# bistoyek21-ric/StrikeForce

Measured on AMD Instinct MI355X. Metric: env-steps/sec (whole node), 64x64 map x32 entities, higher is better.
Workload: dtype int32

## Files before the change

strikeforce_amd/csrc/sf_core.hpp:

```cpp
#pragma once
#include "../../include/strikeforce.h"
#include "sf_types.hpp"

#if defined(SF_EXP_FAKE_DRAWS) && !defined(SF_EXPERIMENT_BUILD)
#error "SF_EXP_FAKE_DRAWS makes draw() return wrong numbers on purpose (tools/experiments/r03_rows): timing builds only, together with -DSF_EXPERIMENT_BUILD"
#endif

namespace sf {

enum { SH_WALL, SH_HUMAN, SH_ZOMBIE, SH_PUP, SH_PDN, SH_BULLET, SH_CHEST, SH_POUT, SH_EMPTY };
enum { LIM_PORTAL = 1000, LIM_BLOCK = 1100 };

#define SF_SHAPE(f) (SH::FIXED ? SH::f(p) : p.f)
constexpr uint32_t mod5_frac(uint32_t x) { return (x * 205u) & 1023u; }
constexpr bool mod5_frac_exact() {
  for (uint32_t x = 0; x < 1024u; ++x)
    if ((x % 5u < 2u) != (mod5_frac(x) < 410u) || (x % 5u < 3u) != (mod5_frac(x) < 615u)) return false;
  return true;
}
static_assert(mod5_frac_exact(), "x % 5 < 2 and x % 5 < 3 by the fraction's bits, for every x < 1024");
#define SF_MOD5_LT(x, n) (SH::FIXED ? mod5_frac(x) < ((n) == 2u ? 410u : 615u) : mod5(x) < (n))
template <class W, int NB, bool HBM_PLANE = false, bool BITMAPS = !HBM_PLANE, bool ZL = false, class SH = RuntimeShape>
struct Core {
  using V = typename W::V;
  using P = typename W::P;

  struct Arena {
    V hpos, hfl, hhp, hst, hmd, hk, hdm, hef, hc01, hc23, ht01, ht23, hbpk, hcmd;
    V zpos, zhp, zmd;
    uint32_t *zl;
    uint32_t zcap;
    uint32_t zwn;
    uint32_t zwhi;
    uint32_t *pl;
    uint32_t pwn, pwhi;
    V ba[NB], bd[NB], bb[NB], bc[NB];
    V ppos;
    V rl, rus, rseed;
    V rl2, rseed2;
    uint32_t warm;
    uint32_t wrate;
    const uint32_t *xt;
    const uint32_t *ht;
    uint32_t *bm;
    V la;
    V la2;
    uint32_t la2_ok;
    int32_t frame, kills, tkills, loot, chests, steps, episodes, done, outcome, ended;
    int32_t fph;
    uint32_t jomle;
    uint32_t tb_lo, tb_hi, sr_lo, sr_hi;
    uint32_t dirty;
    uint32_t pd01, pd23, pd45;
#ifdef SF_DIAG_STAMPS
    V dacc;
    uint32_t dlast;
#endif
  };

  static constexpr uint32_t RL_ZERO = 0x10000u;
  static SF_DEV V mod65537_v(V x) {
    const V t = (x & 0xffffu) - (x >> 16);
    return W::minu(t, t + 65537u);
  }
  static SF_DEV V pow3_v(const uint32_t *xt, V m, P pred) {
    return mod65537_v(W::lds_u32(xt, m & 255u, pred) * W::lds_u32(xt + 256, m >> 8, pred));
  }

  template <bool WANT_OUT>
  static SF_DEV V draw_core(V &rl, const V &rus, const V &rseed, uint32_t &jomle, const uint32_t *xt, const Params &p) {
    const P tap = W::ltu(W::lane(), 18u) & ((rl & RL_ZERO) == 0u);
    const V pw = pow3_v(xt, (rl * rseed) & 0xffffu, tap);
    const V sum = W::sum18_row1(W::select(tap, rus * pw, V(0u))) + 1u;
    V t = mod65537_v(sum);
    t = W::select(t == 0u, V(1u), t);
    jomle += 1u;
    const uint32_t e = jomle & 0xffffu;
    const V lg = W::gload_u16(p.logt, t + (uint32_t)LOGT_OFF, W::all());
    const V lnew = (lg * e) & 0xffffu;
    rl = W::select(W::lane() == 17u, lnew, W::shl1(rl));
    if (WANT_OUT) return pow3_v(xt, lnew, W::all()) & 1023u;
    return V(0u);
  }
  static constexpr uint32_t SUM_BIAS_LANE = 63489u + 11u * 65537u;
  static_assert((32ull * SUM_BIAS_LANE) % 65537ull == 1ull, "the lanes' bias must add up to the generator's +1");
  static_assert(SUM_BIAS_LANE % 2u == 0u, "it is also a byte offset into a table of 16-bit entries");
  static_assert(16ull * SUM_BIAS_LANE > 16ull * 10ull * 65536ull, "a row's partial sum must stay positive");
  static_assert((32ull * SUM_BIAS_LANE + 18ull * 10ull * 65535ull) >> 16 < (unsigned long long)LOGT_OFF, "index below the table");
  static SF_DEV const uint16_t *log_base(const Params &p) { return p.logt + LOGT_OFF - (int)(SUM_BIAS_LANE / 2u); }
  static SF_DEV V issue_offset(const uint32_t *xt, V rl, V rseed, V rus, V &d) {
    const V m = W::mul24(rl, rseed);
    const V pr = W::pow_bytes(xt, m);
    d = (pr & 0xffffu) - (pr >> 16);
    return W::rng_reduce(d, rus, V(SUM_BIAS_LANE));
  }
  static SF_DEV uint32_t draw_issue(Arena &S, const Params &p) {
    V d;
    S.la = W::gload_u16_at(log_base(p), issue_offset(S.xt, S.rl, S.rseed, S.rus, d));
    W::rng_prio_end();
    const int32_t o = (int32_t)W::readlane(d, 18u);
    return (uint32_t)(o + ((o >> 31) & 65537)) & 1023u;
  }
  static SF_DEV uint32_t draw(Arena &S, const uint8_t *, const Params &p) {
#ifdef SF_EXP_FAKE_DRAWS
    S.jomle = S.jomle * 1664525u + 1013904223u;
    return (W::readlane(S.rl, (S.jomle >> 26) & 31u) ^ (S.jomle >> 16)) & 1023u;
#endif
    SF_PROF(PH_RNG);
    S.jomle += 1u;
    if constexpr (W::FUSED_ROUND) {
      uint32_t out;
      const V off = W::rng_round(S.rl, S.jomle, S.la, S.rseed, S.rus, V(SUM_BIAS_LANE), S.xt, out);
      S.la = W::gload_u16_at(log_base(p), off);
      return out;
    }
    S.rl = W::rng_commit(S.rl, S.jomle, S.la);
    return draw_issue(S, p);
  }

  static SF_DEV void seed_digits(V &digits, uint64_t x, uint32_t lane18 = 0u) {
    digits = V(0u);
    W::setlane(digits, 18u, lane18);
    for (int i = 0; i < 18; ++i) {
      W::setlane(digits, (uint32_t)i, (uint32_t)(x % 10u) + 1u);
      x /= 10u;
    }
  }
  static SF_DEV void srand_(Arena &S, const uint8_t *lds, const Params &p, uint64_t tb, uint64_t us) {
    S.rl = V(RL_ZERO);
    seed_digits(S.rus, us);
    seed_digits(S.rseed, tb, 1u);
    S.jomle = 18u;
    (void)lds;
    for (int i = 0; i < 1024; ++i) draw_core<false>(S.rl, S.rus, S.rseed, S.jomle, S.xt, p);
    draw_issue(S, p);
  }
  static SF_DEV void prewarm_issue(Arena &S, const Params &p) {
    V d;
    S.la2 = W::gload_u16_at(log_base(p), issue_offset(S.xt, S.rl2, S.rseed2, S.rus, d));
    S.la2_ok = 1u;
  }
  static SF_DEV void prewarm_one(Arena &S, const Params &p) {
#ifdef SF_EXP_FAKE_DRAWS
    S.warm = 1024u;
    return;
#endif
    SF_PROF(PH_WARM);
    if (S.warm >= 1024u) return;
#ifdef SF_EXP_FREE_WARMUP
    if (S.warm & 3u) {
      ++S.warm;
      return;
    }
#endif
    uint32_t j2 = 18u + S.warm;
    if (S.warm < 18u) {
      draw_core<false>(S.rl2, S.rus, S.rseed2, j2, S.xt, p);
    } else {
      if (!S.la2_ok) prewarm_issue(S, p);
      const V lnew = W::mul24(S.la2, V((j2 + 1u) & 0xffffu)) & 0xffffu;
      S.rl2 = W::select(W::lane() == 17u, lnew, W::shl1(S.rl2));
      S.la2_ok = 0u;
      if (S.warm + 1u < 1024u) prewarm_issue(S, p);
    }
    ++S.warm;
  }
  static SF_DEV void prewarm(Arena &S, const uint8_t *lds, const Params &p, uint32_t n) {
    (void)lds;
    for (; n && S.warm < 1024u; --n) prewarm_one(S, p);
  }

  static SF_DEV int DX(int d) { return d == 0 ? 1 : (d == 2 ? -1 : 0); }
  static SF_DEV int DY(int d) { return d == 1 ? 1 : (d == 3 ? -1 : 0); }
  static SF_DEV uint32_t cellidx(const Params &p, int f, int r, int c) { return (uint32_t)((f * SF_SHAPE(N) + r) * SF_SHAPE(M) + c); }
  static SF_DEV uint32_t cellidx_q(const Params &p, uint32_t q) { return cellidx(p, pos_f(q), pos_r(q), pos_c(q)); }
  static SF_DEV bool inmap(const Params &p, int r, int c) {
    return (uint32_t)r < (uint32_t)SF_SHAPE(N) && (uint32_t)c < (uint32_t)SF_SHAPE(M);
  }
  static SF_DEV uint32_t flags_at(const uint8_t *lds, const Params &p, int f, int r, int c) {
    if (!inmap(p, r, c)) return SF_CELL_WALL;
    return W::ulds_u8(lds, cellidx(p, f, r, c));
  }
  static SF_DEV int human_at(const Arena &S, uint32_t q) {
    uint64_t m = W::ballot(((S.hfl & HF_OCC) != 0u) & (S.hpos == q));
    return m ? W::ctz64(m) : -1;
  }
  static SF_DEV int live_human_at(const Arena &S, uint32_t q) {
    uint64_t m = W::ballot(((S.hfl & HF_ALIVE) != 0u) & (S.hpos == q));
// ... 1430 lines not shown
    if (state != SF_REPLAY_RUNNING || done) return;
    const V fl = W::gload(p.hum, W::lane() + ((uint32_t)HW_FLAGS * (uint32_t)p.A + (uint32_t)a) * (uint32_t)SF_SHAPE(H), ag);
    const P takes = ag & !me & ((fl & (HF_ALIVE | HF_CTRL)) == (HF_ALIVE | HF_CTRL));
    const uint64_t bal = W::ballot(takes);
    const V line = V(cur) + W::rank_below(bal);
    const P have = takes & W::ltu(line, V(len));
    const V tok = W::gload_u8(r.streams, line + o0, have);
    W::gstore_u8(r.cmd, row, tok, have);
    W::gstore_u8(r.taken, row, tok, have);
    const uint32_t want = (uint32_t)W::popc64(bal), left = len - cur, got = want < left ? want : left;
    W::ustore_i32(st + RP_CURSOR, (int32_t)(cur + got));
    if (got < want) W::ustore_i32(st + RP_STATE, SF_REPLAY_TRUNCATED);
  }

  template <bool LOG = false>
  static SF_DEV void loop_top(Arena &S, uint8_t *lds, const Params &p, int a) {
    SF_PROF(PH_TOP);
    spawns(S, lds, p);
    const int out = check_end(S, p);
    if (out != SF_RUNNING) {
      S.done = 1, S.outcome = out;
      latch_results<LOG>(S, p, a);
    }
  }

  static SF_DEV void reset_state(Arena &S, uint8_t *lds, const Params &p, uint64_t tb, uint64_t serial, bool adopt) {
    S.frame = S.kills = S.tkills = S.loot = S.chests = S.steps = 0;
    frame_phases(S);
    S.done = 0, S.outcome = SF_RUNNING;
    S.tb_lo = (uint32_t)tb, S.tb_hi = (uint32_t)(tb >> 32), S.sr_lo = (uint32_t)serial, S.sr_hi = (uint32_t)(serial >> 32);
    S.hpos = V(POS_NONE), S.hfl = V(0u), S.hhp = V(0u), S.hst = V(0u), S.hmd = V(0u), S.hk = V(0u), S.hdm = V(0u);
    S.hef = V(0u), S.hc01 = V(0u), S.hc23 = V(0u), S.ht01 = V(0u), S.ht23 = V(0u), S.hbpk = V(0u);
    S.hcmd = V((uint32_t)'+');
    S.zpos = V(0u), S.zhp = V(0u), S.zmd = V(0u);
    if constexpr (ZL) S.zwn = 0u;
#pragma unroll
    for (int j = 0; j < NB; ++j) S.ba[j] = V(0u), S.bd[j] = V(0u), S.bb[j] = V(0u), S.bc[j] = V(0u);
    if constexpr (ZL) {
      S.ppos = V(0u);
      S.pwn = (uint32_t)p.pw0;
      for (uint32_t j = 0; j < S.pwn; ++j) {
        const V sl = W::lane() + 64u * j;
        W::lds_store_u32(S.pl + 64u * j, W::lane(), W::gload(p.map_exits, sl, W::ltu(sl, (uint32_t)p.P)), W::all());
      }
      if (S.pwhi < S.pwn) S.pwhi = S.pwn;
    } else {
      S.ppos = W::gload(p.map_exits, W::lane(), W::ltu(W::lane(), (uint32_t)p.P));
    }
    W::copy_g2l(lds, p.map_flags, (uint32_t)SF_SHAPE(cells_pad));
    S.dirty = 1u;
    if (adopt) {
      prewarm(S, lds, p, 1024u);
      S.rl = S.rl2, S.rseed = S.rseed2, S.jomle = 18u + 1024u;
      draw_issue(S, p);
    } else {
      srand_(S, lds, p, tb, serial);
    }
    if (SF_SHAPE(auto_reset)) {
      seed_digits(S.rseed2, tb + (uint64_t)(uint32_t)p.reseed, 1u);
      S.rl2 = V(RL_ZERO);
      S.warm = 0u, S.la2_ok = 0u;
    }
    const int count = SF_SHAPE(mode) == SF_MODE_BATTLE ? SF_SHAPE(n_agents) : (SF_SHAPE(mode) == SF_MODE_SQUAD ? 10 : 1);
    SF_NOUNROLL for (int i = 0; i < count; ++i) {
      int prof = 0, team = 1;
      uint32_t q = pos_pack(0, 1, 1), fl = HF_CTRL;
      if (SF_SHAPE(mode) == SF_MODE_BATTLE) {
        q = POS_NONE, team = p.tab->teams[i], fl = HF_CTRL | (i != SF_SHAPE(ind) ? HF_REMOTE : 0u);
      } else if (SF_SHAPE(mode) == SF_MODE_SQUAD) {
        prof = i ? 1 : 0;
        team = i < 5 ? 1 : 2;
        q = i == 0 ? pos_pack(0, 3, 1) : pos_pack(i < 5 ? 0 : p.squad_floor, 1, i + 1);
        fl = (i == 0 || i < SF_SHAPE(n_agents)) ? HF_CTRL : 0u;
      }
      human_make(S, p, (uint32_t)i, prof, q, 1, team, fl, (SF_SHAPE(mode) == SF_MODE_BATTLE && p.npc_block > 1) ? i : 0);
    }
    if (SF_SHAPE(mode) == SF_MODE_BATTLE) {
      S.hfl = S.hfl & ~HF_OCC;
      SF_NOUNROLL for (int i = 0; i < SF_SHAPE(n_agents); ++i) {
        const uint32_t way = draw(S, lds, p) % 4u + 1u;
        SF_NOUNROLL for (int guard = 0; guard < (1 << 20); ++guard) {
          const uint32_t q = draw_cell(S, lds, p);
          uint32_t fl;
          if (showit_q(S, lds, p, q, fl) == SH_EMPTY) {
            W::setlane(S.hpos, (uint32_t)i, q);
            W::setlane(S.hfl, (uint32_t)i, ((W::readlane(S.hfl, (uint32_t)i) & ~HF_WAY_MASK) | way) | HF_OCC);
            break;
          }
        }
      }
    }
  }

  template <int PHASE = 0, bool LOG = false>
  static SF_DEV void step(Arena &S, uint8_t *lds, const Params &p, int a) {
    if (S.done) return;
    SF_STAMP(S, 0);
    uint32_t rest = 0u;
    SF_NOUNROLL for (int half = (PHASE == 2 ? 1 : 0); half < (PHASE == 1 ? 1 : 2); ++half) {
      const uint32_t j0 = S.jomle;
      if (half == 0) {
        zombie_action(S, lds, p);
        SF_STAMP(S, 1);
      } else {
        human_action(S, lds, p, a);
        SF_STAMP(S, 3);
      }
// ... 97 lines not shown
        zl_put(S, ZW_HP, j, W::gload(z + ZW_HP * AZ, sl, in), W::all());
        zl_put(S, ZW_MINDAMAGE, j, W::gload(z + ZW_MINDAMAGE * AZ, sl, in), W::all());
      }
    } else {
      const P in = W::ltu(ln, (uint32_t)SF_SHAPE(Z));
      const uint32_t *z = p.zom + (size_t)a * (size_t)SF_SHAPE(Z);
      S.zpos = W::gload(z + ZW_POS * AZ, ln, in), S.zhp = W::gload(z + ZW_HP * AZ, ln, in);
      S.zmd = W::gload(z + ZW_MINDAMAGE * AZ, ln, in);
    }
#pragma unroll
    for (int j = 0; j < NB; ++j) {
      const V sl = ln + (uint32_t)(64 * j);
      const P in = W::ltu(sl, (uint32_t)SF_SHAPE(B));
      const uint32_t *b = p.bul + (size_t)a * (size_t)SF_SHAPE(B);
      S.ba[j] = W::gload(b + BW_A * AB, sl, in), S.bd[j] = W::gload(b + BW_DAMAGE * AB, sl, in);
      S.bb[j] = W::gload(b + BW_B * AB, sl, in), S.bc[j] = W::gload(b + BW_C * AB, sl, in);
    }
    if constexpr (ZL) {
      S.ppos = V(0u);
      S.pwn = (uint32_t)W::uload_i32(p.scal + (size_t)a * SC_WORDS + SC_PWN);
      if (S.pwn > (uint32_t)zw_for(p.P)) S.pwn = (uint32_t)zw_for(p.P);
      S.pwhi = S.pwn;
      for (uint32_t j = 0; j < S.pwn; ++j) {
        const V sl = ln + 64u * j;
        W::lds_store_u32(S.pl + 64u * j, ln, W::gload(p.por + (size_t)a * (size_t)p.P, sl, W::ltu(sl, (uint32_t)p.P)), W::all());
      }
    } else {
      S.ppos = W::gload(p.por + (size_t)a * (size_t)p.P, ln, W::ltu(ln, (uint32_t)p.P));
    }
    {
      const P in = W::ltu(ln, 18u);
      const V rw = W::gload(p.rng + (size_t)a * RNG_WORDS, ln, in);
      const V val = rw & 0xfffffu;
      S.rus = (rw >> 20) & 15u, S.rseed = W::select(ln == 18u, V(1u), (rw >> 24) & 15u);
        const P nz = in & (val != 0u);
      S.rl = W::select(nz, W::gload_u16(p.logt, val + (uint32_t)LOGT_OFF, nz), V(RL_ZERO));
      const V rw2 = W::gload(p.rng2 + (size_t)a * RNG_WORDS, ln, in);
      S.rl2 = rw2 & 0x1ffffu, S.rseed2 = W::select(ln == 18u, V(1u), rw2 >> 24);
    }
    const V sc = W::gload((const uint32_t *)p.scal + (size_t)a * SC_WORDS, ln, W::ltu(ln, (uint32_t)SC_WORDS));
    S.frame = (int32_t)W::readlane(sc, SC_FRAME), S.kills = (int32_t)W::readlane(sc, SC_KILLS);
    frame_phases(S);
    S.tkills = (int32_t)W::readlane(sc, SC_TKILLS), S.loot = (int32_t)W::readlane(sc, SC_LOOT);
    S.chests = (int32_t)W::readlane(sc, SC_CHESTS), S.jomle = W::readlane(sc, SC_JOMLE);
    S.steps = (int32_t)W::readlane(sc, SC_STEPS), S.episodes = (int32_t)W::readlane(sc, SC_EPISODES);
    S.done = (int32_t)W::readlane(sc, SC_DONE), S.outcome = (int32_t)W::readlane(sc, SC_OUTCOME);
    S.ended = (int32_t)W::readlane(sc, SC_ENDED);
    S.tb_lo = W::readlane(sc, SC_TB_LO), S.tb_hi = W::readlane(sc, SC_TB_HI);
    S.sr_lo = W::readlane(sc, SC_SR_LO), S.sr_hi = W::readlane(sc, SC_SR_HI);
    S.warm = W::readlane(sc, SC_WARM);
    S.pd01 = W::readlane(sc, SC_PD01), S.pd23 = W::readlane(sc, SC_PD23), S.pd45 = W::readlane(sc, SC_PD45);
    if (!HBM_PLANE && copy_plane) W::copy_g2l(lds, p.flags + (size_t)a * (size_t)SF_SHAPE(cells_pad), (uint32_t)SF_SHAPE(cells_pad));
    S.dirty = 0u;
    if (copy_plane) draw_issue(S, p);
  }

  static SF_DEV void store(const Arena &S, const uint8_t *lds, const Params &p, int a) {
    const V ln = W::lane();
    const size_t AH = (size_t)p.A * (size_t)SF_SHAPE(H), AZ = (size_t)p.A * (size_t)SF_SHAPE(Z), AB = (size_t)p.A * (size_t)SF_SHAPE(B);
    {
      const P in = W::ltu(ln, (uint32_t)SF_SHAPE(H));
      uint32_t *h = p.hum + (size_t)a * (size_t)SF_SHAPE(H);
      W::gstore(h + HW_POS * AH, ln, S.hpos, in), W::gstore(h + HW_FLAGS * AH, ln, S.hfl, in);
      W::gstore(h + HW_HP * AH, ln, S.hhp, in), W::gstore(h + HW_STAMINA * AH, ln, S.hst, in);
      W::gstore(h + HW_MINDAMAGE * AH, ln, S.hmd, in), W::gstore(h + HW_KILLS * AH, ln, S.hk, in);
      W::gstore(h + HW_DAMAGE * AH, ln, S.hdm, in), W::gstore(h + HW_EFFECT * AH, ln, S.hef, in);
      W::gstore(h + HW_CONS01 * AH, ln, S.hc01, in), W::gstore(h + HW_CONS23 * AH, ln, S.hc23, in);
      W::gstore(h + HW_THR01 * AH, ln, S.ht01, in), W::gstore(h + HW_THR23 * AH, ln, S.ht23, in);
      W::gstore(h + HW_BPK * AH, ln, S.hbpk, in);
    }
    uint32_t zlive_n = 0u;
    (void)zlive_n;
    if constexpr (ZL) {
      uint32_t *z = p.zom + (size_t)a * (size_t)SF_SHAPE(Z);
      for (uint32_t j = 0; j < S.zwhi; ++j) {
        const V sl = ln + 64u * j;
        const P in = W::ltu(sl, (uint32_t)SF_SHAPE(Z));
        const bool used = j < S.zwn;
        const V zpw = used ? zl_get(S, ZW_POS, j) : V(0u);
        W::gstore(z + ZW_POS * AZ, sl, zpw, in);
        W::gstore(z + ZW_HP * AZ, sl, used ? zl_get(S, ZW_HP, j) : V(0u), in);
        W::gstore(z + ZW_MINDAMAGE * AZ, sl, used ? zl_get(S, ZW_MINDAMAGE, j) : V(0u), in);
        zlive_n += (uint32_t)W::popc64(W::ballot((zpw & ZF_ALIVE) != 0u));
      }
    } else {
      const P in = W::ltu(ln, (uint32_t)SF_SHAPE(Z));
      uint32_t *z = p.zom + (size_t)a * (size_t)SF_SHAPE(Z);
      W::gstore(z + ZW_POS * AZ, ln, S.zpos, in), W::gstore(z + ZW_HP * AZ, ln, S.zhp, in);
      W::gstore(z + ZW_MINDAMAGE * AZ, ln, S.zmd, in);
    }
#pragma unroll
    for (int j = 0; j < NB; ++j) {
      const V sl = ln + (uint32_t)(64 * j);
      const P in = W::ltu(sl, (uint32_t)SF_SHAPE(B));
      uint32_t *b = p.bul + (size_t)a * (size_t)SF_SHAPE(B);
      W::gstore(b + BW_A * AB, sl, S.ba[j], in), W::gstore(b + BW_DAMAGE * AB, sl, S.bd[j], in);
      W::gstore(b + BW_B * AB, sl, S.bb[j], in), W::gstore(b + BW_C * AB, sl, S.bc[j], in);
    }
    if constexpr (ZL) {
      for (uint32_t j = 0; j < S.pwhi; ++j) {
        const V sl = ln + 64u * j;
        W::gstore(p.por + (size_t)a * (size_t)p.P, sl, j < S.pwn ? pl_get(S, j) : V(0u), W::ltu(sl, (uint32_t)p.P));
      }
    } else {
      W::gstore(p.por + (size_t)a * (size_t)p.P, ln, S.ppos, W::ltu(ln, (uint32_t)p.P));
    }
    {
// ... 82 lines not shown
    const bool chosen = (r.mask && mb != 0u) || (r.done_too && done != 0) || (r.max_steps > 0 && done == 0 && steps >= r.max_steps);
    if (r.selected)
      W::gstore_u8(r.selected + (size_t)a * (size_t)SF_SHAPE(n_agents), W::lane(), V(chosen ? 1u : 0u),
                   W::ltu(W::lane(), (uint32_t)SF_SHAPE(n_agents)));
    if (!chosen) return;
    uint64_t tb, serial;
    if (r.tb) {
      tb = r.tb[a], serial = r.serial[a];
    } else {
      tb = (((uint64_t)(uint32_t)W::uload_i32(sc + SC_TB_HI) << 32) | (uint32_t)W::uload_i32(sc + SC_TB_LO)) + (uint64_t)(uint32_t)p.reseed;
      serial = ((uint64_t)(uint32_t)W::uload_i32(sc + SC_SR_HI) << 32) | (uint32_t)W::uload_i32(sc + SC_SR_LO);
    }
    Arena S;
    S.episodes = episodes, S.ended = 0;
    S.pd01 = S.pd23 = S.pd45 = 0u;
    lds = tables(S, lds, p, a);
    S.rl2 = V(RL_ZERO), S.rseed2 = V(0u), S.warm = 0u, S.wrate = 1u;
    if constexpr (ZL) S.zwhi = (uint32_t)zw_for(SF_SHAPE(Z)), S.pwhi = (uint32_t)zw_for(p.P);
    reset_state(S, lds, p, tb, serial, false);
    frame_advance(S);
    loop_top(S, lds, p, a);
    store(S, lds, p, a);
  }

  static SF_DEV void step_body(uint8_t *lds, const Params &p, int a, const uint8_t *cmds, int k) {
    if (p.tab->ep_ring)
      step_body_t<true>(lds, p, a, cmds, k);
    else
      step_body_t<false>(lds, p, a, cmds, k);
  }
  template <bool LOG>
  static SF_DEV void step_body_t(uint8_t *lds, const Params &p, int a, const uint8_t *cmds, int k) {
    Arena S;
    typename W::template G2L<LDS_EXP_BYTES / 1024> q_exp;
    typename W::template G2L<2> q_ht;
    typename W::template G2L<4> q_pl;
    uint8_t *const tab0 = lds;
    const uint32_t ht_n = (uint32_t)p.ht_bytes < 2048u ? (uint32_t)p.ht_bytes : 2048u;
    const uint32_t pl_n = HBM_PLANE ? 0u : ((uint32_t)SF_SHAPE(cells_pad) < 4096u ? (uint32_t)SF_SHAPE(cells_pad) : 4096u);
    const uint8_t *const pl_g = p.flags + (size_t)a * (size_t)SF_SHAPE(cells_pad);
    W::g2l_issue(q_exp, reinterpret_cast<const uint8_t *>(p.exptab), (uint32_t)LDS_EXP_BYTES);
    W::g2l_issue(q_ht, reinterpret_cast<const uint8_t *>(p.tab->hatab), ht_n);
    W::g2l_issue(q_pl, pl_g, pl_n);
    lds = tables(S, lds, p, a, false);
    load(S, lds, p, a, false);
    W::g2l_store(q_exp, tab0, (uint32_t)LDS_EXP_BYTES);
    W::g2l_store(q_ht, tab0 + LDS_EXP_BYTES, ht_n);
    if ((uint32_t)p.ht_bytes > ht_n)
      W::copy_g2l(tab0 + LDS_EXP_BYTES + ht_n, reinterpret_cast<const uint8_t *>(p.tab->hatab) + ht_n, (uint32_t)p.ht_bytes - ht_n);
    if (!HBM_PLANE) {
      W::g2l_store(q_pl, lds, pl_n);
      if ((uint32_t)SF_SHAPE(cells_pad) > pl_n) W::copy_g2l(lds + pl_n, pl_g + pl_n, (uint32_t)SF_SHAPE(cells_pad) - pl_n);
    }
    draw_issue(S, p);
    const P ag = W::ltu(W::lane(), (uint32_t)SF_SHAPE(n_agents));
    S.wrate = 4u;
    S.ended = 0;
    SF_STAMP_LOADED();
    SF_STAMP_BEGIN(S);
    if constexpr (SH::FIXED) {
      const size_t stride = (size_t)p.A * (size_t)SF_SHAPE(n_agents);
      const uint8_t *c = cmds + (size_t)a * (size_t)SF_SHAPE(n_agents);
      const uint8_t *const end = c + (size_t)(k > 0 ? k : 0) * stride;
      for (; c != end && !S.done; c += stride) {
        S.hcmd = W::select(ag, W::gload_u8(c, W::lane(), ag), V((uint32_t)'+'));
        step<0, LOG>(S, lds, p, a);
        if (S.done) restart<LOG>(S, lds, p, a);
      }
    } else {
      for (int s = 0; s < k; ++s) {
        const uint8_t *c = cmds + ((size_t)s * (size_t)p.A + (size_t)a) * (size_t)SF_SHAPE(n_agents);
        S.hcmd = W::select(ag, W::gload_u8(c, W::lane(), ag), V((uint32_t)'+'));
        step<0, LOG>(S, lds, p, a);
      }
    }
    SF_STAMP_END(S, a);
    SF_STAMP_STEPPED();
    store(S, lds, p, a);
  }

  static SF_DEV void step_half_body(uint8_t *lds, const Params &p, int a, const uint8_t *cmds, int phase) {
    Arena S;
    lds = tables(S, lds, p, a);
    load(S, lds, p, a);
    S.wrate = 4u;
    S.ended = 0;
    SF_STAMP_BEGIN(S);
    if (phase == 1) {
      S.hcmd = V((uint32_t)'+');
      step<1>(S, lds, p, a);
    } else {
      const P ag = W::ltu(W::lane(), (uint32_t)SF_SHAPE(n_agents));
      S.hcmd = W::select(ag, W::gload_u8(cmds + (size_t)a * (size_t)SF_SHAPE(n_agents), W::lane(), ag), V((uint32_t)'+'));
      step<2>(S, lds, p, a);
    }
    SF_STAMP_END(S, a);
    store(S, lds, p, a);
  }
};
#undef SF_SHAPE
#undef SF_FRAME_MOD
#undef SF_MOD5_LT

}
```

strikeforce_amd/csrc/wave_gfx950.hpp:

```cpp
#pragma once
#include <hip/hip_runtime.h>
#include <stdint.h>

#define SF_DEV __device__ __forceinline__

#if (defined(SF_EXP_SHORT_ROUND) || defined(SF_EXP_FREE_WARMUP) || defined(SF_EXP_ZLOOP_FREE)) && !defined(SF_EXPERIMENT_BUILD)
#error "timing experiments (wrong results by construction): only together with -DSF_EXPERIMENT_BUILD"
#endif

namespace sf {

#define SF_GLOBAL __attribute__((address_space(1)))
template <class T>
static __device__ __forceinline__ const SF_GLOBAL T *gptr(const T *p) {
  return (const SF_GLOBAL T *)p;
}
template <class T>
static __device__ __forceinline__ SF_GLOBAL T *gptr(T *p) {
  return (SF_GLOBAL T *)p;
}

typedef uint32_t u32x4 __attribute__((ext_vector_type(4)));

#define SF_COUNT(k)
#define SF_PROF(ph)

#ifdef SF_DIAG_STAMPS
extern __device__ uint32_t sf_diag_buffer[];
#define SF_STAMP_BEGIN(S) ((S).dacc = 0u, (S).dlast = (uint32_t)__builtin_amdgcn_s_memtime())
#define SF_STAMP(S, ph)                                                              \
  do {                                                                               \
    const uint32_t t_ = (uint32_t)__builtin_amdgcn_s_memtime();                      \
    (S).dacc = threadIdx.x == (ph) ? (S).dacc + (t_ - (S).dlast) : (S).dacc;         \
    (S).dlast = t_;                                                                  \
  } while (0)
#define SF_STAMP_END(S, a) \
  do {                     \
    if (threadIdx.x < 16u) ::sf::sf_diag_buffer[(size_t)(a) * 16u + threadIdx.x] = (S).dacc; \
  } while (0)
extern __device__ unsigned long long sf_diag_times[];
#define SF_STAMP_LOADED()                                                                    \
  do {                                                                                       \
    __builtin_amdgcn_s_waitcnt(0);                                                           \
    if (threadIdx.x == 0) ::sf::sf_diag_times[4 * blockIdx.x + 1] = __builtin_amdgcn_s_memrealtime(); \
  } while (0)
#define SF_STAMP_STEPPED()                                                                   \
  do {                                                                                       \
    if (threadIdx.x == 0) ::sf::sf_diag_times[4 * blockIdx.x + 2] = __builtin_amdgcn_s_memrealtime(); \
  } while (0)
#else
#define SF_STAMP_BEGIN(S)
#define SF_STAMP(S, ph)
#define SF_STAMP_END(S, a)
#define SF_STAMP_LOADED()
#define SF_STAMP_STEPPED()
#endif

#ifndef SF_RNG_PRIO
#define SF_RNG_PRIO 1
#endif
#ifndef SF_RNG_PRIO_LEVEL
#define SF_RNG_PRIO_LEVEL 3
#endif
#define SF_STR2(x) #x
#define SF_STR(x) SF_STR2(x)

struct WaveGfx950 {
  using V = uint32_t;
  using P = bool;

  static SF_DEV V lane() { return threadIdx.x; }
  static SF_DEV uint64_t ballot(P p) { return __builtin_amdgcn_ballot_w64(p); }
  static SF_DEV int ctz64(uint64_t m) { return __builtin_ctzll(m); }
  static SF_DEV int clz64(uint64_t m) { return __builtin_clzll(m); }
  static SF_DEV uint32_t uni(uint32_t x) { return (uint32_t)__builtin_amdgcn_readfirstlane((int)x); }
  static SF_DEV uint32_t readlane(const V &v, uint32_t idx) {
    return (uint32_t)__builtin_amdgcn_readlane((int)v, (int)uni(idx));
  }
  static SF_DEV void setlane(V &v, uint32_t idx, uint32_t val) {
    v = (lane() == uni(idx)) ? val : v;
  }
  static SF_DEV V select(P p, V a, V b) { return p ? a : b; }
  static SF_DEV V sar31(V v) { return (uint32_t)((int32_t)v >> 31); }
  static SF_DEV P le0(V v) { return (int32_t)v <= 0; }
  static SF_DEV P ltu(V a, V b) { return a < b; }
  static SF_DEV P frombits(uint64_t m) { return (m >> lane()) & 1ull; }
  static SF_DEV P all() { return true; }
  static SF_DEV V sum18_row1(V v) {
    int x = (int)v;
    x += __builtin_amdgcn_update_dpp(0, x, 0xB1, 0xf, 0xf, true);
    x += __builtin_amdgcn_update_dpp(0, x, 0x4E, 0xf, 0xf, true);
    x += __builtin_amdgcn_update_dpp(0, x, 0x141, 0xf, 0xf, true);
    x += __builtin_amdgcn_update_dpp(0, x, 0x140, 0xf, 0xf, true);
    x += __builtin_amdgcn_update_dpp(0, x, 0x142, 0x2, 0xf, false);
    return (uint32_t)x;
  }
  static SF_DEV V minu(V a, V b) { return a < b ? a : b; }
  static SF_DEV V shrv(V a, V sh) { return a >> sh; }
  static SF_DEV V shlv(V a, V sh) { return a << sh; }
  static SF_DEV P gts(V a, V b) { return (int32_t)a > (int32_t)b; }
  static SF_DEV int popc64(uint64_t m) { return __builtin_popcountll(m); }
  static SF_DEV void lds_or_u32(uint32_t *base, V widx, V bits, P pred) {
    if (pred) (void)__hip_atomic_fetch_or(base + widx, bits, __ATOMIC_RELAXED, __HIP_MEMORY_SCOPE_WORKGROUP);
    __builtin_amdgcn_wave_barrier();
  }
  static SF_DEV V lds_or_rtn_u32(uint32_t *base, V widx, V bits, P pred) {
    uint32_t old = 0u;
    if (pred) old = __hip_atomic_fetch_or(base + widx, bits, __ATOMIC_RELAXED, __HIP_MEMORY_SCOPE_WORKGROUP);
    __builtin_amdgcn_wave_barrier();
    return old;
  }
  static SF_DEV void lds_store_u32(uint32_t *base, V widx, V val, P pred) {
    if (pred) base[widx] = val;
    __builtin_amdgcn_wave_barrier();
  }
  static SF_DEV void lds_zero(uint32_t *base, uint32_t nwords) {
    for (uint32_t off = lane() * 4u; off < nwords; off += 64u * 4u)
      *reinterpret_cast<u32x4 *>(base + off) = (u32x4)(0u);
    __builtin_amdgcn_wave_barrier();
  }
  static SF_DEV V mad24(V a, uint32_t b, V c) { return __umul24(a, b) + c; }
  static SF_DEV void lds_store_u8(uint8_t *lds, V idx, V val, P pred) {
    if (pred) lds[idx] = (uint8_t)val;
    __builtin_amdgcn_wave_barrier();
  }
  static SF_DEV V mul24(V a, V b) {
    uint32_t r;
    asm("v_mul_u32_u24 %0, %1, %2" : "=v"(r) : "v"(a), "v"(b));
    return r;
  }
  static SF_DEV V shl1(V v) { return (uint32_t)__builtin_amdgcn_update_dpp(0, (int)v, 0x130, 0xf, 0xf, true); }

  static SF_DEV V lds_u8(const uint8_t *lds, V idx, P pred) { return pred ? (uint32_t)lds[idx] : 0u; }
  static SF_DEV V lds_u8_any(const uint8_t *lds, V idx) { return (uint32_t)lds[idx]; }
  static SF_DEV uint32_t ulds_u8(const uint8_t *lds, uint32_t idx) { return uni((uint32_t)lds[idx]); }
  static SF_DEV V lds_u32(const uint32_t *lds, V idx, P pred) { return pred ? lds[idx] : 0u; }
  static SF_DEV uint32_t ulds_u32(const uint32_t *lds, uint32_t idx) { return uni(lds[idx]); }
  static SF_DEV void ulds_store_u32(uint32_t *lds, uint32_t idx, uint32_t val) {
    lds[idx] = val;
    __builtin_amdgcn_wave_barrier();
  }
  static SF_DEV V mul24_su(uint32_t a, V b) {
    uint32_t r;
    asm("v_mul_u32_u24 %0, %1, %2" : "=v"(r) : "s"(a), "v"(b));
    return r;
  }
  static SF_DEV void rng_prio_end() {
#if SF_RNG_PRIO == 2
    __builtin_amdgcn_s_setprio(0);
#endif
  }
  static SF_DEV V rng_commit(V rl, uint32_t e, V la) {
    uint32_t t;
    asm volatile(
#if SF_RNG_PRIO
        "s_setprio " SF_STR(SF_RNG_PRIO_LEVEL) "\n\t"
#endif
        "v_mul_u32_u24 %[t], %[e], %[la]\n\t"
        "s_mov_b64 vcc, 0x60000\n\t"
        "v_cndmask_b32_dpp %[rl], %[rl], %[t], vcc wave_shl:1 row_mask:0xf bank_mask:0xf bound_ctrl:1"
        : [rl] "+v"(rl), [t] "=&v"(t)
        : [e] "s"(e), [la] "v"(la)
        : "vcc");
    return rl;
  }
  static SF_DEV V rng_reduce(V d, V us, V bias) {
    uint32_t x;
    asm volatile("v_mad_i32_i24 %[x], %[d], %[us], %[bias]\n\t"
        "s_nop 1\n\t"
#ifndef SF_EXP_SHORT_ROUND
        "v_add_u32_dpp %[x], %[x], %[x] quad_perm:[1,0,3,2] row_mask:0xf bank_mask:0xf\n\t"
        "s_nop 1\n\t"
        "v_add_u32_dpp %[x], %[x], %[x] quad_perm:[2,3,0,1] row_mask:0xf bank_mask:0xf\n\t"
        "s_nop 1\n\t"
        "v_add_u32_dpp %[x], %[x], %[x] row_half_mirror row_mask:0xf bank_mask:0xf\n\t"
        "s_nop 1\n\t"
        "v_add_u32_dpp %[x], %[x], %[x] row_mirror row_mask:0xf bank_mask:0xf\n\t"
        "s_nop 1\n\t"
#endif
        "v_add_u32_dpp %[x], %[x], %[x] row_bcast:15 row_mask:0x2 bank_mask:0xf\n\t"
        "v_sub_u32_sdwa %[x], %[x], %[x] dst_sel:DWORD dst_unused:UNUSED_PAD src0_sel:WORD_0 src1_sel:WORD_1\n\t"
        "v_lshl_add_u32 %[x], %[x], 1, %[bias]"
#if SF_RNG_PRIO == 1
        "\n\ts_setprio 0"
#endif
        : [x] "=&v"(x)
        : [d] "v"(d), [us] "v"(us), [bias] "v"(bias));
    return x;
  }
  static constexpr bool FUSED_ROUND = true;
  static SF_DEV V rng_round(V &rl, uint32_t e, V la, V seed, V us, V bias, const uint32_t *xt, uint32_t &out) {
    typedef const __attribute__((address_space(3))) uint32_t *lptr;
    const uint32_t base = (uint32_t)(uintptr_t)(lptr)xt;
    uint32_t t, m, oa, ob;
    asm volatile(
#if SF_RNG_PRIO
        "s_setprio " SF_STR(SF_RNG_PRIO_LEVEL) "\n\t"
#endif
        "v_mul_u32_u24 %[t], %[e], %[la]\n\t"
        "s_mov_b64 vcc, 0x60000\n\t"
        "v_cndmask_b32_dpp %[rl], %[rl], %[t], vcc wave_shl:1 row_mask:0xf bank_mask:0xf bound_ctrl:1\n\t"
        "v_mul_u32_u24 %[m], %[rl], %[seed]\n\t"
        "v_lshlrev_b32_sdwa %[oa], 2, %[m] dst_sel:DWORD dst_unused:UNUSED_PAD src0_sel:DWORD src1_sel:BYTE_0\n\t"
        "v_lshlrev_b32_sdwa %[ob], 2, %[m] dst_sel:DWORD dst_unused:UNUSED_PAD src0_sel:DWORD src1_sel:BYTE_1"
        : [rl] "+v"(rl), [t] "=&v"(t), [m] "=&v"(m), [oa] "=&v"(oa), [ob] "=&v"(ob)
        : [e] "s"(e), [la] "v"(la), [seed] "v"(seed)
        : "vcc");
    const uint32_t a = *(lptr)(uintptr_t)(oa | base);
    const uint32_t b = *((lptr)(uintptr_t)(ob | base) + 256);
    uint32_t pr, d, x, o, sg;
    asm volatile(
        "v_mul_u32_u24 %[pr], %[a], %[b]\n\t"
        "v_sub_u32_sdwa %[d], %[pr], %[pr] dst_sel:DWORD dst_unused:UNUSED_PAD src0_sel:WORD_0 src1_sel:WORD_1\n\t"
        "v_mad_i32_i24 %[x], %[d], %[us], %[bias]\n\t"
        "v_readlane_b32 %[o], %[d], 18\n\t"
        "s_lshr_b32 %[sg], %[o], 31\n\t"
#ifndef SF_EXP_SHORT_ROUND
        "v_add_u32_dpp %[x], %[x], %[x] quad_perm:[1,0,3,2] row_mask:0xf bank_mask:0xf\n\t"
#endif
        "s_add_i32 %[o], %[o], %[sg]\n\t"
        "s_and_b32 %[o], %[o], 0x3ff\n\t"
#ifndef SF_EXP_SHORT_ROUND
        "v_add_u32_dpp %[x], %[x], %[x] quad_perm:[2,3,0,1] row_mask:0xf bank_mask:0xf\n\t"
        "s_nop 1\n\t"
        "v_add_u32_dpp %[x], %[x], %[x] row_half_mirror row_mask:0xf bank_mask:0xf\n\t"
        "s_nop 1\n\t"
        "v_add_u32_dpp %[x], %[x], %[x] row_mirror row_mask:0xf bank_mask:0xf\n\t"
#endif
        "s_nop 1\n\t"
        "v_add_u32_dpp %[x], %[x], %[x] row_bcast:15 row_mask:0x2 bank_mask:0xf\n\t"
        "v_sub_u32_sdwa %[x], %[x], %[x] dst_sel:DWORD dst_unused:UNUSED_PAD src0_sel:WORD_0 src1_sel:WORD_1\n\t"
        "v_lshl_add_u32 %[x], %[x], 1, %[bias]"
#if SF_RNG_PRIO
        "\n\ts_setprio 0"
#endif
        : [pr] "=&v"(pr), [d] "=&v"(d), [x] "=&v"(x), [o] "=&s"(o), [sg] "=&s"(sg)
        : [a] "v"(a), [b] "v"(b), [us] "v"(us), [bias] "v"(bias)
        : "scc");
    out = o;
    return x;
  }
  static SF_DEV V pow_bytes(const uint32_t *xt, V m) {
    typedef const __attribute__((address_space(3))) uint32_t *lptr;
    const uint32_t base = (uint32_t)(uintptr_t)(lptr)xt;
    uint32_t oa, ob;
    asm("v_lshlrev_b32_sdwa %0, 2, %1 dst_sel:DWORD dst_unused:UNUSED_PAD src0_sel:DWORD src1_sel:BYTE_0" : "=v"(oa) : "v"(m));
    asm("v_lshlrev_b32_sdwa %0, 2, %1 dst_sel:DWORD dst_unused:UNUSED_PAD src0_sel:DWORD src1_sel:BYTE_1" : "=v"(ob) : "v"(m));
    const uint32_t a = *(lptr)(uintptr_t)(oa | base);
    const uint32_t b = *((lptr)(uintptr_t)(ob | base) + 256);
    return mul24(a, b);
  }
  static SF_DEV V pow_pair(const uint32_t *xt, V m4) {
    typedef const __attribute__((address_space(3))) uint32_t *lptr;
    const uint32_t base = (uint32_t)(uintptr_t)(lptr)xt;
    const uint32_t a = *(lptr)(uintptr_t)((m4 & 0x3fcu) | base);
    const uint32_t b = *((lptr)(uintptr_t)(((m4 >> 8) & 0x3fcu) | base) + 256);
    return mul24(a, b);
  }
  static SF_DEV V gload_u16_at(const uint16_t *base, V byte_off) {
    return (uint32_t) * reinterpret_cast<const SF_GLOBAL uint16_t *>(reinterpret_cast<const SF_GLOBAL char *>(gptr(base)) + byte_off);
  }
  static SF_DEV void ulds_store_u8(uint8_t *lds, uint32_t idx, uint32_t val) {
    lds[idx] = (uint8_t)val;
    __builtin_amdgcn_wave_barrier();
  }

  static SF_DEV int32_t uload_i32(const int32_t *p) {
    return (int32_t)uni((uint32_t)__hip_atomic_load(gptr(p), __ATOMIC_RELAXED, __HIP_MEMORY_SCOPE_WAVEFRONT));
  }
  static SF_DEV void ustore_i32(int32_t *p, int32_t v) {
    if (lane() == 0u) __hip_atomic_store(gptr(p), v, __ATOMIC_RELAXED, __HIP_MEMORY_SCOPE_WAVEFRONT);
  }
  static SF_DEV V gload_u16(const uint16_t *base, V idx, P pred) { return pred ? (uint32_t)gptr(base)[idx] : 0u; }
  static SF_DEV int32_t uload_i16(const int16_t *p) {
    return (int32_t)(int16_t)uni((uint32_t)(uint16_t)__hip_atomic_load(gptr(p), __ATOMIC_RELAXED, __HIP_MEMORY_SCOPE_WAVEFRONT));
  }
  static SF_DEV void ustore_i16(int16_t *p, int16_t v) {
    if (lane() == 0u) __hip_atomic_store(gptr(p), v, __ATOMIC_RELAXED, __HIP_MEMORY_SCOPE_WAVEFRONT);
  }

  static SF_DEV V gload(const uint32_t *base, V idx, P pred) { return pred ? gptr(base)[idx] : 0u; }
// ... 49 lines not shown
```

Measured before the change: 239.2 million.

## Replace per-draw cross-lane reduction with running-sum RNG in upper wave lanes

For fixed-shape builds, the random generator keeps a sliding set of partial sums in lanes 46-63 instead of recomputing an 18-term cross-lane reduction on every draw. Each draw now adds one new term to all pending sums with a single wave-shift DPP add and reads the finished sum from lane 46. This removes the chain of dependent DPP adds and nops from the hot draw path. In exchange, the window has to be rebuilt whenever generator state is loaded, seeded or adopted (reversed seed digits via bpermute plus 18 term updates), which adds correctness risk in lane bookkeeping. The SHORT_ROUND experiment flag is also removed.

```diff
diff --git a/strikeforce_amd/csrc/sf_core.hpp b/strikeforce_amd/csrc/sf_core.hpp
--- a/strikeforce_amd/csrc/sf_core.hpp
+++ b/strikeforce_amd/csrc/sf_core.hpp
@@ -20,6 +20,8 @@
 }
 static_assert(mod5_frac_exact(), "x % 5 < 2 and x % 5 < 3 by the fraction's bits, for every x < 1024");
 #define SF_MOD5_LT(x, n) (SH::FIXED ? mod5_frac(x) < ((n) == 2u ? 410u : 615u) : mod5(x) < (n))
+template <class W>
+struct RsRound;
 template <class W, int NB, bool HBM_PLANE = false, bool BITMAPS = !HBM_PLANE, bool ZL = false, class SH = RuntimeShape>
 struct Core {
   using V = typename W::V;
@@ -101,6 +103,65 @@
     const int32_t o = (int32_t)W::readlane(d, 18u);
     return (uint32_t)(o + ((o >> 31) & 65537)) & 1023u;
   }
+  static constexpr uint32_t RS_L0 = 46u, RS_OUT = 45u;
+  static constexpr uint32_t RS_ONE = 180u * 65537u + 1u;
+  static_assert(RS_ONE % 65537u == 1u, "the generator's +1");
+  static_assert(RS_ONE >= 18ull * 10ull * 65535ull, "the complete sum must be positive");
+  static_assert((RS_ONE + 18ull * 10ull * 65535ull) >> 16 < (unsigned long long)LOGT_OFF, "index below the table");
+  static_assert(SUM_BIAS_LANE / 2u >= ((RS_ONE + 18ull * 10ull * 65535ull) >> 16), "the byte offset stays non-negative");
+  static_assert(RS_L0 + 17u == 63u && RS_OUT < RS_L0 && RS_OUT > 18u, "new sums enter from beyond lane 63; the tap-order digits stay clear");
+  static SF_DEV V rs_term(const Arena &S, V l) {
+    const V pr = W::pow_bytes(S.xt, W::mul24(l, S.rseed));
+    return (pr & 0xffffu) - (pr >> 16);
+  }
+  static SF_DEV P rs_rows() { return W::ltu(V(31u), W::lane()); }
+  static SF_DEV void rs_issue(Arena &S, const Params &p) {
+    if constexpr (W::FUSED_ROUND) {
+      S.la = W::gload_u16_at(log_base(p), RsRound<W>::template offset<RS_ONE>(S.rl, V(SUM_BIAS_LANE)));
+      return;
+    }
+    const uint32_t x = W::readlane(S.rl, RS_L0) + RS_ONE;
+    S.la = W::gload_u16_at(log_base(p), V((((x & 0xffffu) - (x >> 16)) << 1) + SUM_BIAS_LANE));
+  }
+  static SF_DEV void rs_rebuild(Arena &S, const Params &p) {
+    if constexpr (W::FUSED_ROUND) {
+      RsRound<W>::reverse(S.rseed, S.rus, W::lane());
+      RsRound<W>::clear(S.rl);
+      _Pragma("clang loop unroll(full)") for (uint32_t q = 0; q < 18u; q += 3u)
+        RsRound<W>::update3(S.rl, W::readlane(S.rl, q), W::readlane(S.rl, q + 1u), W::readlane(S.rl, q + 2u), S.rseed, S.rus, S.xt);
+    } else {
+      const P hi = rs_rows();
+      W::setlane(S.rseed, RS_OUT, 1u), W::setlane(S.rus, RS_OUT, 0u);
+      for (uint32_t q = 0; q < 18u; ++q) {
+        W::setlane(S.rseed, 63u - q, W::readlane(S.rseed, q));
+        W::setlane(S.rus, 63u - q, W::readlane(S.rus, q));
+      }
+      S.rl = W::select(hi, V(0u), S.rl);
+      for (uint32_t q = 0; q < 18u; ++q)
+        S.rl = W::select(hi, W::shl1(S.rl) + rs_term(S, V(W::readlane(S.rl, q))) * S.rus, S.rl);
+    }
+    rs_issue(S, p);
+  }
+  static SF_DEV uint32_t draw_rs(Arena &S, const Params &p) {
+    if constexpr (W::FUSED_ROUND) {
+      uint32_t out;
+      const V off = RsRound<W>::template round<RS_ONE>(S.rl, S.jomle, S.la, S.rseed, S.rus, V(SUM_BIAS_LANE), S.xt, out);
+      S.la = W::gload_u16_at(log_base(p), off);
+      return out;
+    }
+    const V d = rs_term(S, W::mul24(S.la, V(S.jomle & 0xffffu)));
+    S.rl = W::rng_commit(S.rl, S.jomle, S.la);
+    S.rl = S.rl + W::select(rs_rows(), d * S.rus, V(0u));
+    const int32_t o = (int32_t)W::readlane(d, RS_OUT);
+    rs_issue(S, p);
+    return (uint32_t)(o + ((o >> 31) & 65537)) & 1023u;
+  }
+  static SF_DEV void draw_first(Arena &S, const Params &p) {
+    if constexpr (SH::FIXED)
+      rs_rebuild(S, p);
+    else
+      draw_issue(S, p);
+  }
   static SF_DEV uint32_t draw(Arena &S, const uint8_t *, const Params &p) {
 #ifdef SF_EXP_FAKE_DRAWS
     S.jomle = S.jomle * 1664525u + 1013904223u;
@@ -108,6 +169,7 @@
 #endif
     SF_PROF(PH_RNG);
     S.jomle += 1u;
+    if constexpr (SH::FIXED) return draw_rs(S, p);
     if constexpr (W::FUSED_ROUND) {
       uint32_t out;
       const V off = W::rng_round(S.rl, S.jomle, S.la, S.rseed, S.rus, V(SUM_BIAS_LANE), S.xt, out);
@@ -133,7 +195,7 @@
     S.jomle = 18u;
     (void)lds;
     for (int i = 0; i < 1024; ++i) draw_core<false>(S.rl, S.rus, S.rseed, S.jomle, S.xt, p);
-    draw_issue(S, p);
+    draw_first(S, p);
   }
   static SF_DEV void prewarm_issue(Arena &S, const Params &p) {
     V d;
@@ -1670,7 +1732,7 @@
     if (adopt) {
       prewarm(S, lds, p, 1024u);
       S.rl = S.rl2, S.rseed = S.rseed2, S.jomle = 18u + 1024u;
-      draw_issue(S, p);
+      draw_first(S, p);
     } else {
       srand_(S, lds, p, tb, serial);
     }
@@ -1874,7 +1936,7 @@
     S.pd01 = W::readlane(sc, SC_PD01), S.pd23 = W::readlane(sc, SC_PD23), S.pd45 = W::readlane(sc, SC_PD45);
     if (!HBM_PLANE && copy_plane) W::copy_g2l(lds, p.flags + (size_t)a * (size_t)SF_SHAPE(cells_pad), (uint32_t)SF_SHAPE(cells_pad));
     S.dirty = 0u;
-    if (copy_plane) draw_issue(S, p);
+    if (copy_plane) draw_first(S, p);
   }
 
   static SF_DEV void store(const Arena &S, const uint8_t *lds, const Params &p, int a) {
@@ -2063,7 +2125,7 @@
       W::g2l_store(q_pl, lds, pl_n);
       if ((uint32_t)SF_SHAPE(cells_pad) > pl_n) W::copy_g2l(lds + pl_n, pl_g + pl_n, (uint32_t)SF_SHAPE(cells_pad) - pl_n);
     }
-    draw_issue(S, p);
+    draw_first(S, p);
     const P ag = W::ltu(W::lane(), (uint32_t)SF_SHAPE(n_agents));
     S.wrate = 4u;
     S.ended = 0;
diff --git a/strikeforce_amd/csrc/wave_gfx950.hpp b/strikeforce_amd/csrc/wave_gfx950.hpp
--- a/strikeforce_amd/csrc/wave_gfx950.hpp
+++ b/strikeforce_amd/csrc/wave_gfx950.hpp
@@ -4,7 +4,7 @@
 
 #define SF_DEV __device__ __forceinline__
 
-#if (defined(SF_EXP_SHORT_ROUND) || defined(SF_EXP_FREE_WARMUP) || defined(SF_EXP_ZLOOP_FREE)) && !defined(SF_EXPERIMENT_BUILD)
+#if (defined(SF_EXP_FREE_WARMUP) || defined(SF_EXP_ZLOOP_FREE)) && !defined(SF_EXPERIMENT_BUILD)
 #error "timing experiments (wrong results by construction): only together with -DSF_EXPERIMENT_BUILD"
 #endif
 
@@ -65,6 +65,139 @@
 #define SF_STR2(x) #x
 #define SF_STR(x) SF_STR2(x)
 
+template <class W>
+struct RsRound;
+struct WaveGfx950;
+template <>
+struct RsRound<WaveGfx950> {
+  template <uint32_t ONE>
+  static __device__ __forceinline__ uint32_t round(uint32_t &rl, uint32_t e, uint32_t la, uint32_t seed, uint32_t us, uint32_t offc, const uint32_t *xt, uint32_t &out) {
+    typedef const __attribute__((address_space(3))) uint32_t *lptr;
+    const uint32_t base = (uint32_t)(uintptr_t)(lptr)xt;
+    uint32_t es;
+    asm("v_mul_u32_u24 %0, %1, %2" : "=v"(es) : "s"(e), "v"(seed));
+    uint32_t oa, ob;
+    asm volatile(
+#if SF_RNG_PRIO
+        "s_setprio " SF_STR(SF_RNG_PRIO_LEVEL) "\n\t"
+#endif
+        "v_mul_u32_u24 %[oa], %[la], %[es]\n\t"
+        "v_lshlrev_b32_sdwa %[ob], 2, %[oa] dst_sel:DWORD dst_unused:UNUSED_PAD src0_sel:DWORD src1_sel:BYTE_1\n\t"
+        "v_lshlrev_b32_sdwa %[oa], 2, %[oa] dst_sel:DWORD dst_unused:UNUSED_PAD src0_sel:DWORD src1_sel:BYTE_0"
+        : [oa] "=&v"(oa), [ob] "=&v"(ob)
+        : [la] "v"(la), [es] "v"(es));
+    uint32_t a = *(lptr)(uintptr_t)(oa | base);
+    uint32_t b = *((lptr)(uintptr_t)(ob | base) + 256);
+    rl = commit(rl, e, la);
+    uint32_t sx, o;
+    asm volatile(
+        "v_mul_u32_u24 %[a], %[a], %[b]\n\t"
+        "v_sub_u32_sdwa %[a], %[a], %[a] dst_sel:DWORD dst_unused:UNUSED_PAD src0_sel:WORD_0 src1_sel:WORD_1\n\t"
+        "v_mul_i32_i24 %[b], %[a], %[us]\n\t"
+        "v_add_u32_dpp %[rl], %[rl], %[b] wave_shl:1 row_mask:0xc bank_mask:0xf bound_ctrl:1\n\t"
+        "v_readlane_b32 %[o], %[a], 45\n\t"
+        "v_readlane_b32 %[sx], %[rl], 46\n\t"
+        "s_add_u32 %[sx], %[sx], %[one]\n\t"
+        "s_cmp_lt_i32 %[o], 0\n\t"
+        "v_sub_u32_sdwa %[b], %[sx], %[sx] dst_sel:DWORD dst_unused:UNUSED_PAD src0_sel:WORD_0 src1_sel:WORD_1\n\t"
+        "s_addc_u32 %[o], %[o], 0\n\t"
+        "v_lshl_add_u32 %[b], %[b], 1, %[offc]\n\t"
+        "s_and_b32 %[o], %[o], 0x3ff"
+#if SF_RNG_PRIO
+        "\n\ts_setprio 0"
+#endif
+        : [rl] "+v"(rl), [a] "+v"(a), [b] "+v"(b), [sx] "=&s"(sx), [o] "=&s"(o)
+        : [us] "v"(us), [offc] "v"(offc), [one] "n"(ONE)
+        : "scc");
+    out = o;
+    return b;
+  }
+  static __device__ __forceinline__ void update3(uint32_t &rl, uint32_t l0, uint32_t l1, uint32_t l2, uint32_t seed, uint32_t us,
+                                                 const uint32_t *xt) {
+    typedef const __attribute__((address_space(3))) uint32_t *lptr;
+    const uint32_t base = (uint32_t)(uintptr_t)(lptr)xt;
+    uint32_t oa0, ob0, oa1, ob1, oa2, ob2;
+    asm volatile(
+        "v_mul_u32_u24 %[oa0], %[l0], %[seed]\n\t"
+        "v_lshlrev_b32_sdwa %[ob0], 2, %[oa0] dst_sel:DWORD dst_unused:UNUSED_PAD src0_sel:DWORD src1_sel:BYTE_1\n\t"
+        "v_lshlrev_b32_sdwa %[oa0], 2, %[oa0] dst_sel:DWORD dst_unused:UNUSED_PAD src0_sel:DWORD src1_sel:BYTE_0\n\t"
+        "v_mul_u32_u24 %[oa1], %[l1], %[seed]\n\t"
+        "v_lshlrev_b32_sdwa %[ob1], 2, %[oa1] dst_sel:DWORD dst_unused:UNUSED_PAD src0_sel:DWORD src1_sel:BYTE_1\n\t"
+        "v_lshlrev_b32_sdwa %[oa1], 2, %[oa1] dst_sel:DWORD dst_unused:UNUSED_PAD src0_sel:DWORD src1_sel:BYTE_0\n\t"
+        "v_mul_u32_u24 %[oa2], %[l2], %[seed]\n\t"
+        "v_lshlrev_b32_sdwa %[ob2], 2, %[oa2] dst_sel:DWORD dst_unused:UNUSED_PAD src0_sel:DWORD src1_sel:BYTE_1\n\t"
+        "v_lshlrev_b32_sdwa %[oa2], 2, %[oa2] dst_sel:DWORD dst_unused:UNUSED_PAD src0_sel:DWORD src1_sel:BYTE_0"
+        : [oa0] "=&v"(oa0), [ob0] "=&v"(ob0), [oa1] "=&v"(oa1), [ob1] "=&v"(ob1), [oa2] "=&v"(oa2), [ob2] "=&v"(ob2)
+        : [l0] "s"(l0), [l1] "s"(l1), [l2] "s"(l2), [seed] "v"(seed));
+    uint32_t a0 = *(lptr)(uintptr_t)(oa0 | base), b0 = *((lptr)(uintptr_t)(ob0 | base) + 256);
+    uint32_t a1 = *(lptr)(uintptr_t)(oa1 | base), b1 = *((lptr)(uintptr_t)(ob1 | base) + 256);
+    uint32_t a2 = *(lptr)(uintptr_t)(oa2 | base), b2 = *((lptr)(uintptr_t)(ob2 | base) + 256);
+    asm volatile(
+        "v_mul_u32_u24 %[a0], %[a0], %[b0]\n\t"
+        "v_sub_u32_sdwa %[a0], %[a0], %[a0] dst_sel:DWORD dst_unused:UNUSED_PAD src0_sel:WORD_0 src1_sel:WORD_1\n\t"
+        "v_mul_i32_i24 %[b0], %[a0], %[us]\n\t"
+        "v_add_u32_dpp %[rl], %[rl], %[b0] wave_shl:1 row_mask:0xc bank_mask:0xf bound_ctrl:1\n\t"
+        "v_mul_u32_u24 %[a1], %[a1], %[b1]\n\t"
+        "v_sub_u32_sdwa %[a1], %[a1], %[a1] dst_sel:DWORD dst_unused:UNUSED_PAD src0_sel:WORD_0 src1_sel:WORD_1\n\t"
+        "v_mul_i32_i24 %[b1], %[a1], %[us]\n\t"
+        "v_add_u32_dpp %[rl], %[rl], %[b1] wave_shl:1 row_mask:0xc bank_mask:0xf bound_ctrl:1\n\t"
+        "v_mul_u32_u24 %[a2], %[a2], %[b2]\n\t"
+        "v_sub_u32_sdwa %[a2], %[a2], %[a2] dst_sel:DWORD dst_unused:UNUSED_PAD src0_sel:WORD_0 src1_sel:WORD_1\n\t"
+        "v_mul_i32_i24 %[b2], %[a2], %[us]\n\t"
+        "v_add_u32_dpp %[rl], %[rl], %[b2] wave_shl:1 row_mask:0xc bank_mask:0xf bound_ctrl:1"
+        : [rl] "+v"(rl), [a0] "+v"(a0), [b0] "+v"(b0), [a1] "+v"(a1), [b1] "+v"(b1), [a2] "+v"(a2), [b2] "+v"(b2)
+        : [us] "v"(us));
+  }
+  template <uint32_t ONE>
+  static __device__ __forceinline__ uint32_t offset(uint32_t rl, uint32_t offc) {
+    uint32_t b, sx;
+    asm volatile(
+        "v_readlane_b32 %[sx], %[rl], 46\n\t"
+        "s_add_u32 %[sx], %[sx], %[one]\n\t"
+        "s_nop 0\n\t"
+        "v_sub_u32_sdwa %[b], %[sx], %[sx] dst_sel:DWORD dst_unused:UNUSED_PAD src0_sel:WORD_0 src1_sel:WORD_1\n\t"
+        "v_lshl_add_u32 %[b], %[b], 1, %[offc]"
+        : [b] "=&v"(b), [sx] "=&s"(sx)
+        : [rl] "v"(rl), [offc] "v"(offc), [one] "n"(ONE)
+        : "scc");
+    return b;
+  }
+  static __device__ __forceinline__ void clear(uint32_t &rl) {
+    asm volatile("s_mov_b64 vcc, 0xffffffff\n\t"
+                 "v_cndmask_b32 %[rl], 0, %[rl], vcc"
+                 : [rl] "+v"(rl)
+                 :
+                 : "vcc");
+  }
+  static __device__ __forceinline__ void reverse(uint32_t &seed, uint32_t &us, uint32_t lane) {
+    uint32_t a, s2, u2;
+    asm volatile(
+        "v_sub_u32 %[a], 63, %[lane]\n\t"
+        "v_lshlrev_b32 %[a], 2, %[a]\n\t"
+        "ds_bpermute_b32 %[s2], %[a], %[seed]\n\t"
+        "ds_bpermute_b32 %[u2], %[a], %[us]\n\t"
+        "s_mov_b32 vcc_lo, 0\n\t"
+        "s_mov_b32 vcc_hi, 0xffffe000\n\t"
+        "s_waitcnt lgkmcnt(0)\n\t"
+        "v_cndmask_b32 %[seed], %[seed], %[s2], vcc\n\t"
+        "v_cndmask_b32 %[us], %[us], %[u2], vcc"
+        : [seed] "+v"(seed), [us] "+v"(us), [a] "=&v"(a), [s2] "=&v"(s2), [u2] "=&v"(u2)
+        : [lane] "v"(lane)
+        : "vcc");
+  }
+  static __device__ __forceinline__ uint32_t commit(uint32_t rl, uint32_t e, uint32_t la) {
+    uint32_t t;
+    asm volatile(
+        "v_mul_u32_u24 %[t], %[e], %[la]\n\t"
+        "s_mov_b64 vcc, 0x60000\n\t"
+        "v_cndmask_b32_dpp %[rl], %[rl], %[t], vcc wave_shl:1 row_mask:0x3 bank_mask:0xf bound_ctrl:1"
+        : [rl] "+v"(rl), [t] "=&v"(t)
+        : [e] "s"(e), [la] "v"(la)
+        : "vcc");
+    return rl;
+  }
+};
+
 struct WaveGfx950 {
   using V = uint32_t;
   using P = bool;
@@ -168,7 +301,6 @@
     uint32_t x;
     asm volatile("v_mad_i32_i24 %[x], %[d], %[us], %[bias]\n\t"
         "s_nop 1\n\t"
-#ifndef SF_EXP_SHORT_ROUND
         "v_add_u32_dpp %[x], %[x], %[x] quad_perm:[1,0,3,2] row_mask:0xf bank_mask:0xf\n\t"
         "s_nop 1\n\t"
         "v_add_u32_dpp %[x], %[x], %[x] quad_perm:[2,3,0,1] row_mask:0xf bank_mask:0xf\n\t"
@@ -177,7 +309,6 @@
         "s_nop 1\n\t"
         "v_add_u32_dpp %[x], %[x], %[x] row_mirror row_mask:0xf bank_mask:0xf\n\t"
         "s_nop 1\n\t"
-#endif
         "v_add_u32_dpp %[x], %[x], %[x] row_bcast:15 row_mask:0x2 bank_mask:0xf\n\t"
         "v_sub_u32_sdwa %[x], %[x], %[x] dst_sel:DWORD dst_unused:UNUSED_PAD src0_sel:WORD_0 src1_sel:WORD_1\n\t"
         "v_lshl_add_u32 %[x], %[x], 1, %[bias]"
@@ -215,18 +346,14 @@
         "v_mad_i32_i24 %[x], %[d], %[us], %[bias]\n\t"
         "v_readlane_b32 %[o], %[d], 18\n\t"
         "s_lshr_b32 %[sg], %[o], 31\n\t"
-#ifndef SF_EXP_SHORT_ROUND
         "v_add_u32_dpp %[x], %[x], %[x] quad_perm:[1,0,3,2] row_mask:0xf bank_mask:0xf\n\t"
-#endif
         "s_add_i32 %[o], %[o], %[sg]\n\t"
         "s_and_b32 %[o], %[o], 0x3ff\n\t"
-#ifndef SF_EXP_SHORT_ROUND
         "v_add_u32_dpp %[x], %[x], %[x] quad_perm:[2,3,0,1] row_mask:0xf bank_mask:0xf\n\t"
         "s_nop 1\n\t"
         "v_add_u32_dpp %[x], %[x], %[x] row_half_mirror row_mask:0xf bank_mask:0xf\n\t"
         "s_nop 1\n\t"
         "v_add_u32_dpp %[x], %[x], %[x] row_mirror row_mask:0xf bank_mask:0xf\n\t"
-#endif
         "s_nop 1\n\t"
         "v_add_u32_dpp %[x], %[x], %[x] row_bcast:15 row_mask:0x2 bank_mask:0xf\n\t"
         "v_sub_u32_sdwa %[x], %[x], %[x] dst_sel:DWORD dst_unused:UNUSED_PAD src0_sel:WORD_0 src1_sel:WORD_1\n\t"
```

After: 250.7 million, median of 6. 4.8% higher.
